# eggsbenedicto/DiffusionRenderer-ComfyUI

Measured on AMD Instinct MI355X. Metric: denoising_steps_per_sec, higher is better.
Workload: dtype bf16; 1 GPU; inverse pass, 57f x 576 x 1024 clip: EDM Euler step = 1 DiT forward (D=4096, 28 blocks, 32 heads) over S=18432 tokens, guidance 0; parallelism=sp1 (token bands; self-attention exchange: none), weights=random-init (hash generator), 7.2e9 params bf16

## Files before the change

diffusionrenderer-comfyui_amd/csrc/attention16.hip:

```cpp
#include "drn_common.h"
#include "drn_launchers.h"
#include "mx_quant.h"

#define QROWS 256
#define KVT 64
#define KBYTES (KVT * 256)
#define NKB 3
#define NVB 4
#ifndef RESCALE_THR
#define RESCALE_THR 6.0f
#endif

typedef const __attribute__((address_space(1))) void* gptr_t;
typedef __attribute__((address_space(3))) void* lptr_t;

template <bool MX>
__global__ __launch_bounds__(512, 2) void attention16_fwd_kernel(
    const bf16_t* __restrict__ Q, const bf16_t* __restrict__ Kp, const bf16_t* __restrict__ Vp, bf16_t* __restrict__ O,
    int heads, int64_t Sq, int64_t Sk_total, int64_t ldq, int64_t ldk, int64_t ldv, int64_t ldo, int64_t bsq, int64_t bsk,
    int64_t bsv, int64_t bso, float scale_log2e, int nqb, int total, int nsplit, int64_t kv_chunk,
    float* __restrict__ Opart, float* __restrict__ MLpart, uint8_t* __restrict__ OQ, uint8_t* __restrict__ OS, int64_t mx_bs) {
    __shared__ __attribute__((aligned(1024))) char smem[(NKB + NVB) * KBYTES];

    const int tid = threadIdx.x;
    const int lane = tid & 63;
    const int wave = __builtin_amdgcn_readfirstlane(tid >> 6);
    const int c = lane & 15, g = lane >> 4;

    int pid;
    {
        const int bid = blockIdx.x;
        const int q = total >> 3, r = total & 7, xcd = bid & 7;
        pid = (xcd < r ? xcd * (q + 1) : r * (q + 1) + (xcd - r) * q) + (bid >> 3);
    }
    const int qb = pid % nqb;
    const int rest = pid / nqb;
    const int split = rest % nsplit;
    const int bh = rest / nsplit;
    const int b = bh / heads, head = bh - b * heads;
    const int64_t q0 = (int64_t)qb * QROWS + wave * 32;
    const int64_t kv_begin = (int64_t)split * kv_chunk;
    const int64_t Sk = min(kv_chunk, Sk_total - kv_begin);

    const bf16_t* Qb = Q + b * bsq + (int64_t)head * 128;
    const bf16_t* Kb = Kp + b * bsk + kv_begin * ldk + (int64_t)head * 128;
    const bf16_t* Vb = Vp + b * bsv + kv_begin * ldv + (int64_t)head * 128;

    bf16x8_t qf[2][4];
#pragma unroll
    for (int qt = 0; qt < 2; ++qt) {
        int64_t qrow = q0 + 16 * qt + c;
        if (qrow > Sq - 1) qrow = Sq - 1;
        const bf16_t* qp = Qb + qrow * ldq + 8 * g;
#pragma unroll
        for (int ks = 0; ks < 4; ++ks) qf[qt][ks] = *reinterpret_cast<const bf16x8_t*>(qp + 32 * ks);
    }
#pragma unroll
    for (int qt = 0; qt < 2; ++qt)
#pragma unroll
        for (int ks = 0; ks < 4; ++ks) asm volatile("" : "+v"(qf[qt][ks]));

    int st_row[2], st_kc[2], st_vc[2];
#pragma unroll
    for (int i = 0; i < 2; ++i) {
        st_row[i] = 4 * (2 * wave + i) + (lane >> 4);
        const int cp = lane & 15;
        st_kc[i] = (cp ^ (st_row[i] & 15)) * 8;
        st_vc[i] = (cp ^ (((st_row[i] & 3) << 1) | (((st_row[i] >> 3) & 1) << 3))) * 8;
    }
    const int dma_off = wave * 2048;
    uint32_t kso[2], vso[2];
#pragma unroll
    for (int i = 0; i < 2; ++i) {
        kso[i] = 2u * (uint32_t)(st_row[i] * (int)ldk + st_kc[i]);
// ... 1 lines not shown
    }
    const int last_rows = (int)(Sk - (int64_t)((Sk - 1) / KVT) * KVT);
#define CLAMP_LAST_TILE()                                                                     \
    do {                                                                                      \
        _Pragma("unroll") for (int i = 0; i < 2; ++i) {                                       \
            const int r_ = min(st_row[i], last_rows - 1);                                     \
            kso[i] = 2u * (uint32_t)(r_ * (int)ldk + st_kc[i]);                               \
            vso[i] = 2u * (uint32_t)(r_ * (int)ldv + st_vc[i]);                               \
        }                                                                                     \
    } while (0)
#define DMA16(SRC, DST) __builtin_amdgcn_global_load_lds((gptr_t)(SRC), (lptr_t)(DST), 16, 0, 0)
#define DMA_PIECE_AT(P, KPTR, VPTR, KBUF, VBUF)                                               \
    do {                                                                                      \
        if ((P) & 1) DMA16((VPTR) + vso[(P) >> 1], smem + (NKB + (VBUF)) * KBYTES + dma_off + ((P) >> 1) * 1024); \
        else DMA16((KPTR) + kso[(P) >> 1], smem + (KBUF) * KBYTES + dma_off + ((P) >> 1) * 1024); \
    } while (0)
#define DMA_WAIT(N) asm volatile("s_waitcnt vmcnt(%0)" :: "i"(N) : "memory")
#define FENCE() __builtin_amdgcn_sched_barrier(0)
#define BARRIER()                                                                             \
    do {                                                                                      \
        FENCE();                                                                              \
        __builtin_amdgcn_s_barrier();                                                         \
        FENCE();                                                                              \
    } while (0)

    const uint32_t lds0 = (uint32_t)(uintptr_t)((lptr_t)smem);
    const int pc = (c & 3) | ((c & 4) << 1) | ((c & 8) >> 1);
    uint32_t ka[4];
#pragma unroll
    for (int ks = 0; ks < 4; ++ks) ka[ks] = lds0 + pc * 256 + (((4 * ks + g) ^ pc) << 4);
    const int vq = c >> 2, vp = c & 3;
    const int kap = ((g & 1) << 3) | ((g & 2) << 1);
    uint32_t va[8];
#pragma unroll
    for (int dt = 0; dt < 8; ++dt)
        va[dt] = lds0 + NKB * KBYTES + (kap + vq) * 256 + 32 * (dt ^ (vq | ((g & 1) << 2))) + 16 * (vp >> 1) + 8 * (vp & 1);

    f32x4_t acc[8][2];
#pragma unroll
    for (int dt = 0; dt < 8; ++dt)
#pragma unroll
        for (int qt = 0; qt < 2; ++qt) acc[dt][qt] = f32x4_t{0.f, 0.f, 0.f, 0.f};
    float m_run[2] = {-INFINITY, -INFINITY}, l_run[2] = {0.f, 0.f};
    f32x4_t lacc[2] = {f32x4_t{0.f, 0.f, 0.f, 0.f}, f32x4_t{0.f, 0.f, 0.f, 0.f}};
    bf16x8_t ones_frag;
#pragma unroll
    for (int i = 0; i < 8; ++i) ones_frag[i] = (short)0x3f80;
    asm volatile("" : "+v"(ones_frag));
    f32x4_t sacc[4][2];
    bf16x8_t pb[2][2] = {};

    bf16x8_t kring[8];
    struct vfrag_t { bf16x4_t lo, hi; } vring[8];
#define RD_K(F16, SLOT)                                                             \
    asm volatile("ds_read_b128 %0, %1 offset:%2" : "=v"(kring[SLOT]) : "v"(ka[(F16) & 3]), "i"(((F16) >> 2) * 4096) : "memory")
#define RD_V(F16, SLOT)                                              \
    asm volatile("ds_read_b64_tr_b16 %0, %2 offset:%3\n\tds_read_b64_tr_b16 %1, %2 offset:%4"                         \
                 : "=&v"(vring[SLOT].lo), "=&v"(vring[SLOT].hi)                                                       \
                 : "v"(va[(F16) & 7]), "i"((32 * ((F16) >> 3)) * 256), "i"((32 * ((F16) >> 3) + 16) * 256) : "memory")
#ifndef ATT16_TIE
#define ATT16_TIE 0
#endif
#if ATT16_TIE
#define WAIT_K(N, SLOT) asm volatile("s_waitcnt lgkmcnt(%1)" : "+v"(kring[SLOT]) : "i"(N) : "memory")
#define WAIT_V(N, SLOT) asm volatile("s_waitcnt lgkmcnt(%2)" : "+v"(vring[SLOT].lo), "+v"(vring[SLOT].hi) : "i"(N) : "memory")
#else
#define WAIT_K(N, SLOT) asm volatile("s_waitcnt lgkmcnt(%0)" :: "i"(N) : "memory")
#define WAIT_V(N, SLOT) asm volatile("s_waitcnt lgkmcnt(%0)" :: "i"(N) : "memory")
#endif
#define JOIN(X) __builtin_shufflevector(X.lo, X.hi, 0, 1, 2, 3, 4, 5, 6, 7)
#define MFMA16(A, B, C) __builtin_amdgcn_mfma_f32_16x16x32_bf16(A, B, C, 0, 0, 0)
#define ISSUE(F)                                                                              \
    do {                                                                                      \
        if ((F) < 16) RD_V(F, (F) & 7);                                                       \
        else if ((F) < 32) RD_K((F) - 16, (F) & 7);                                           \
        else RD_V((F) - 32, (F) & 7);                                                         \
    } while (0)
#define NV_(F) ((F) < 16 ? 2 : ((F) < 32 ? 1 : 2))
#define PEND(F) (NV_((F) + 1) + NV_((F) + 2) + NV_((F) + 3) + NV_((F) + 4) + NV_((F) + 5) + NV_((F) + 6) + NV_((F) + 7))
#ifndef ATT16_PAIR
#define ATT16_PAIR 0
#endif
#ifndef ATT16_DMA_IN_S
#define ATT16_DMA_IN_S 0
#endif
#ifndef ATT16_LSUM_MFMA
#define ATT16_LSUM_MFMA 1
#endif
#ifndef ATT16_PRIO
#define ATT16_PRIO 1
#endif
#ifndef ATT16_SPRIO
#define ATT16_SPRIO 0
#endif
#ifndef ATT16_BAR1
#define ATT16_BAR1 0
#endif
#ifndef ATT16_ABL
#define ATT16_ABL 0
#endif
#define PAIRED(F, PENDING) (ATT16_PAIR && !ATT16_TIE ? (((F) & 1) ? -1 : (PENDING) - NV_((F) + 1)) : (PENDING))
#define STEP_PV(F, PENDING, NEXT)                                                             \
    do {                                                                                      \
        if (PAIRED(F, PENDING) >= 0) WAIT_V(PAIRED(F, PENDING), (F) & 7);                     \
        FENCE();                                                                              \
        {                                                                                     \
            const bf16x8_t vf_ = JOIN(vring[(F) & 7]);                                        \
            acc[(F) & 7][0] = MFMA16(vf_, pb[(F) >> 3][0], acc[(F) & 7][0]);                  \
            acc[(F) & 7][1] = MFMA16(vf_, pb[(F) >> 3][1], acc[(F) & 7][1]);                  \
            if (ATT16_LSUM_MFMA && ((F) & 7) == 4) {        \
                lacc[0] = MFMA16(ones_frag, pb[(F) >> 3][0], lacc[0]);                        \
                lacc[1] = MFMA16(ones_frag, pb[(F) >> 3][1], lacc[1]);                        \
            }                                                                                 \
        }                                                                                     \
        if (NEXT) ISSUE((F) + 8);                                                             \
        FENCE();                                                                              \
    } while (0)
#define STEP_QK(F, PENDING)                                                                   \
    do {                                                                                      \
        if (PAIRED(F, PENDING) >= 0) WAIT_K(PAIRED(F, PENDING), (F) & 7);                     \
        FENCE();                                                                              \
        if ((((F) - 16) & 3) == 0) {                                                          \
            sacc[((F) - 16) >> 2][0] = MFMA16(kring[(F) & 7], qf[0][0], (f32x4_t{0.f, 0.f, 0.f, 0.f})); \
            sacc[((F) - 16) >> 2][1] = MFMA16(kring[(F) & 7], qf[1][0], (f32x4_t{0.f, 0.f, 0.f, 0.f})); \
        } else {                                                                              \
            sacc[((F) - 16) >> 2][0] = MFMA16(kring[(F) & 7], qf[0][((F) - 16) & 3], sacc[((F) - 16) >> 2][0]); \
            sacc[((F) - 16) >> 2][1] = MFMA16(kring[(F) & 7], qf[1][((F) - 16) & 3], sacc[((F) - 16) >> 2][1]); \
        }                                                                                     \
        ISSUE((F) + 8);                                                                       \
        FENCE();                                                                              \
    } while (0)
#define K_STEP(DELTA) do { _Pragma("unroll") for (int ks = 0; ks < 4; ++ks) ka[ks] += (DELTA); } while (0)
#define V_STEP(DELTA) do { _Pragma("unroll") for (int dt = 0; dt < 8; ++dt) va[dt] += (DELTA); } while (0)

#define QK_MASK(T)                                                                            \
    do {                                                                                      \
        if ((int64_t)((T) + 1) * KVT > Sk) {                                                  \
            const int64_t kbase = (int64_t)(T) * KVT + kap;                                   \
            _Pragma("unroll") for (int kt = 0; kt < 4; ++kt)                                  \
                _Pragma("unroll") for (int i = 0; i < 4; ++i)                                 \
                    if (kbase + 16 * kt + i >= Sk) { sacc[kt][0][i] = -INFINITY; sacc[kt][1][i] = -INFINITY; } \
        }                                                                                     \
    } while (0)

#define MAX3(A, B, C) __builtin_fmaxf(__builtin_fmaxf(A, B), C)
#define SOFTMAX_PHASE()                                                                       \
    do {                                                                                      \
        float mx[2];                                                                          \
        {    \
            float a0[2], a2[2];                                                               \
            _Pragma("unroll") for (int qt = 0; qt < 2; ++qt) {                                \
                float b0 = MAX3(sacc[0][qt][0], sacc[0][qt][1], sacc[0][qt][2]);              \
                float b1 = MAX3(sacc[0][qt][3], sacc[1][qt][0], sacc[1][qt][1]);              \
                float b2 = MAX3(sacc[1][qt][2], sacc[1][qt][3], sacc[2][qt][0]);              \
                float b3 = MAX3(sacc[2][qt][1], sacc[2][qt][2], sacc[2][qt][3]);              \
                float b4 = MAX3(sacc[3][qt][0], sacc[3][qt][1], sacc[3][qt][2]);              \
                a0[qt] = MAX3(b0, b1, sacc[3][qt][3]);                                        \
                a2[qt] = MAX3(b2, b3, b4);                                                    \
            }                                                                                 \
            uint32_t u0 = __float_as_uint(fmaxf(a0[0], a2[0])), u1 = __float_as_uint(fmaxf(a0[1], a2[1])); \
            auto s0 = __builtin_amdgcn_permlane32_swap(u0, u0, false, false);       \
            auto s1 = __builtin_amdgcn_permlane32_swap(u1, u1, false, false);                 \
            u0 = __float_as_uint(fmaxf(__uint_as_float(s0[0]), __uint_as_float(s0[1])));      \
            u1 = __float_as_uint(fmaxf(__uint_as_float(s1[0]), __uint_as_float(s1[1])));      \
            s0 = __builtin_amdgcn_permlane16_swap(u0, u0, false, false);            \
            s1 = __builtin_amdgcn_permlane16_swap(u1, u1, false, false);                      \
            mx[0] = fmaxf(__uint_as_float(s0[0]), __uint_as_float(s0[1]));                    \
            mx[1] = fmaxf(__uint_as_float(s1[0]), __uint_as_float(s1[1]));                    \
        }                                                                                     \
         \
        if (__any(mx[0] > m_thr[0] || mx[1] > m_thr[1])) {                                    \
            _Pragma("unroll") for (int qt = 0; qt < 2; ++qt) {                                \
                const float m_new = fmaxf(m_run[qt], mx[qt]);                                 \
                const float alpha = __builtin_amdgcn_exp2f((m_run[qt] - m_new) * scale_log2e); \
                m_run[qt] = m_new;                                                            \
                m_thr[qt] = m_new + thr_raw;                                                  \
                mcs[qt] = m_new * scale_log2e;                                                \
                l_run[qt] *= alpha;                                                           \
                lacc[qt] *= alpha;                                                            \
                _Pragma("unroll") for (int dt = 0; dt < 8; ++dt) acc[dt][qt] *= alpha;        \
            }                                                                                 \
        }                                                                                     \
        _Pragma("unroll") for (int qt = 0; qt < 2; ++qt) {                                    \
            const float mc = mcs[qt];                                                         \
            float ps[2] = {0.f, 0.f};                                                         \
            _Pragma("unroll") for (int s_ = 0; s_ < 2; ++s_) {                                \
                float p[8];                                                                   \
                _Pragma("unroll") for (int j = 0; j < 8; ++j) {                               \
                    if (ATT16_ABL & 1) p[j] = sacc[2 * s_ + (j >> 2)][qt][j & 3] * scale_log2e - mc;      \
                    else p[j] = __builtin_amdgcn_exp2f(sacc[2 * s_ + (j >> 2)][qt][j & 3] * scale_log2e - mc); \
                    if (!ATT16_LSUM_MFMA) ps[j & 1] += p[j];                                  \
                }                                                                             \
                union { bf16x8_t v; uint32_t u[4]; } cv;                                      \
                _Pragma("unroll") for (int i = 0; i < 4; ++i) cv.u[i] = pack_bf2(p[2 * i], p[2 * i + 1]); \
                pb[s_][qt] = cv.v;                                                            \
            }                                                                                 \
            if (!ATT16_LSUM_MFMA) l_run[qt] += ps[0] + ps[1];                                 \
        }                                                                                     \
    } while (0)

    const float thr_raw = RESCALE_THR / scale_log2e;
    float m_thr[2] = {-INFINITY, -INFINITY}, mcs[2] = {0.f, 0.f};
    const int nt = (int)((Sk + KVT - 1) / KVT);
    const int grp = wave >> 2;
    if (nt == 1 && last_rows < KVT) CLAMP_LAST_TILE();
    {
        const char* k0_ = reinterpret_cast<const char*>(Kb);
        const char* v0_ = reinterpret_cast<const char*>(Vb);
        DMA_PIECE_AT(0, k0_, v0_, 0, 0); DMA_PIECE_AT(1, k0_, v0_, 0, 0); DMA_PIECE_AT(2, k0_, v0_, 0, 0); DMA_PIECE_AT(3, k0_, v0_, 0, 0);
    }
    const int64_t ktile_bytes = (int64_t)KVT * ldk * 2, vtile_bytes = (int64_t)KVT * ldv * 2;
    if (nt > 1) {
        if (nt == 2 && last_rows < KVT) CLAMP_LAST_TILE();
        const char* k1_ = reinterpret_cast<const char*>(Kb) + ktile_bytes;
        const char* v1_ = reinterpret_cast<const char*>(Vb) + vtile_bytes;
        DMA_PIECE_AT(0, k1_, v1_, 1, 1); DMA_PIECE_AT(1, k1_, v1_, 1, 1); DMA_PIECE_AT(2, k1_, v1_, 1, 1); DMA_PIECE_AT(3, k1_, v1_, 1, 1);
    }
    DMA_WAIT(0);
    BARRIER();
    if (nt == 3 && last_rows < KVT) CLAMP_LAST_TILE();
    if (!ATT16_BAR1 && grp == 1) BARRIER();
    const char* kreq_p = reinterpret_cast<const char*>(Kb) + (int64_t)min(2, nt - 1) * ktile_bytes;
    const char* vreq_p = reinterpret_cast<const char*>(Vb) + (int64_t)min(2, nt - 1) * vtile_bytes;
    int kbuf = 0, vbuf = 0;
    int kreq = 2 % NKB, vreq = 2 % NVB;
#define REQ_PIECE_NOW(P)                                                                      \
    do {                                                                                      \
        if (!(ATT16_ABL & 4)) DMA_PIECE_AT(P, kreq_p, vreq_p, kreq, vreq);                    \
        FENCE();                                                                              \
    } while (0)
#define REQ_PIECE(P) do { if (!ATT16_DMA_IN_S) REQ_PIECE_NOW(P); } while (0)
#define AFTER_REQUESTS(T)                                                                     \
    do {                                                                                      \
        kreq = kreq == NKB - 1 ? 0 : kreq + 1;                                                \
        vreq = vreq == NVB - 1 ? 0 : vreq + 1;                                                \
        if ((T) + 3 == nt - 1 && last_rows < KVT) CLAMP_LAST_TILE();     \
        if (!(ATT16_ABL & 8) && (T) + 3 <= nt - 1) { kreq_p += ktile_bytes; vreq_p += vtile_bytes; }    \
    } while (0)
#define M_QK(T)                                                                               \
    do {                                                                                      \
        STEP_QK(16, PEND(16)); STEP_QK(17, PEND(17)); STEP_QK(18, PEND(18)); STEP_QK(19, PEND(19)); \
        REQ_PIECE(2);                                                                         \
        STEP_QK(20, PEND(20)); STEP_QK(21, PEND(21)); STEP_QK(22, PEND(22)); STEP_QK(23, PEND(23)); \
        K_STEP(kbuf == NKB - 1 ? -(NKB - 1) * KBYTES : KBYTES);                               \
        kbuf = kbuf == NKB - 1 ? 0 : kbuf + 1;                                                \
        STEP_QK(24, PEND(24)); STEP_QK(25, PEND(25)); STEP_QK(26, PEND(26)); STEP_QK(27, PEND(27)); \
        REQ_PIECE(3);                                                                         \
        STEP_QK(28, PEND(28)); STEP_QK(29, PEND(29)); STEP_QK(30, PEND(30)); STEP_QK(31, PEND(31)); \
        QK_MASK(T);                                                                           \
        if (!ATT16_DMA_IN_S) AFTER_REQUESTS(T);                                               \
        FENCE();                                                                              \
        __builtin_amdgcn_s_setprio(ATT16_SPRIO);                                              \
         \
        if (!ATT16_BAR1 || grp == 1) {                                                        \
            if (ATT16_DMA_IN_S) DMA_WAIT(0); else DMA_WAIT(4);                                \
            BARRIER();                                                                        \
        }                                                                                     \
    } while (0)
#define S_SEGMENT(T)                                                                          \
    do {                                                                                      \
        if (ATT16_DMA_IN_S) {                                                                 \
            REQ_PIECE_NOW(0); REQ_PIECE_NOW(1); REQ_PIECE_NOW(2); REQ_PIECE_NOW(3);           \
            AFTER_REQUESTS(T);                                                                \
        }                                                                                     \
        if (!(ATT16_ABL & 2)) SOFTMAX_PHASE();                                                \
        else { _Pragma("unroll") for (int kt = 0; kt < 4; ++kt) asm volatile("" :: "v"(sacc[kt][0]), "v"(sacc[kt][1])); } \
        FENCE();                                                                              \
         \
        asm volatile("" : "+v"(pb[0][0]), "+v"(pb[0][1]), "+v"(pb[1][0]), "+v"(pb[1][1]), "+v"(l_run[0]), "+v"(l_run[1]) :: "memory"); \
        if (!ATT16_BAR1) BARRIER();                                                           \
        else if (grp == 0) { DMA_WAIT(4); BARRIER(); }                                        \
    } while (0)

    __builtin_amdgcn_s_setprio(ATT16_PRIO);
    ISSUE(16); ISSUE(17); ISSUE(18); ISSUE(19); ISSUE(20); ISSUE(21); ISSUE(22); ISSUE(23);
    FENCE();
    REQ_PIECE(0);
    REQ_PIECE(1);
    M_QK(0);
    S_SEGMENT(0);
    for (int t = 1; t < nt; ++t) {
        __builtin_amdgcn_s_setprio(ATT16_PRIO);
        STEP_PV(0, PEND(0), 1); STEP_PV(1, PEND(1), 1); STEP_PV(2, PEND(2), 1); STEP_PV(3, PEND(3), 1);
        REQ_PIECE(0);
        STEP_PV(4, PEND(4), 1); STEP_PV(5, PEND(5), 1); STEP_PV(6, PEND(6), 1); STEP_PV(7, PEND(7), 1);
        V_STEP(vbuf == NVB - 1 ? -(NVB - 1) * KBYTES : KBYTES);
        vbuf = vbuf == NVB - 1 ? 0 : vbuf + 1;
        STEP_PV(8, PEND(8), 1); STEP_PV(9, PEND(9), 1); STEP_PV(10, PEND(10), 1); STEP_PV(11, PEND(11), 1);
        REQ_PIECE(1);
        STEP_PV(12, PEND(12), 1); STEP_PV(13, PEND(13), 1); STEP_PV(14, PEND(14), 1); STEP_PV(15, PEND(15), 1);
        M_QK(t);
        S_SEGMENT(t);
    }
    __builtin_amdgcn_s_setprio(ATT16_PRIO);
    STEP_PV(0, 14, 1); STEP_PV(1, 14, 1); STEP_PV(2, 14, 1); STEP_PV(3, 14, 1);
    STEP_PV(4, 14, 1); STEP_PV(5, 14, 1); STEP_PV(6, 14, 1); STEP_PV(7, 14, 1);
    STEP_PV(8, 14, 0); STEP_PV(9, 12, 0); STEP_PV(10, 10, 0); STEP_PV(11, 8, 0);
    STEP_PV(12, 6, 0); STEP_PV(13, 4, 0); STEP_PV(14, 2, 0); STEP_PV(15, 0, 0);
    __builtin_amdgcn_s_setprio(0);
    DMA_WAIT(0);
    if (!ATT16_BAR1 && grp == 0) BARRIER();

    float l_tot[2];
#pragma unroll
    for (int qt = 0; qt < 2; ++qt) {
        if (ATT16_LSUM_MFMA) {
            l_tot[qt] = lacc[qt][0];
        } else {
            float l = l_run[qt] + __shfl_xor(l_run[qt], 16, 64);
            l_tot[qt] = l + __shfl_xor(l, 32, 64);
        }
    }
    if (nsplit > 1) {
        const int nbatch = total / (nqb * heads * nsplit);
#pragma unroll
        for (int qt = 0; qt < 2; ++qt) {
            const int64_t qrow = q0 + 16 * qt + c;
            if (qrow < Sq) {
                const int64_t rowid = ((int64_t)split * nbatch + b) * Sq + qrow;
                float* op = Opart + rowid * ((int64_t)heads * 128) + (int64_t)head * 128 + 4 * g;
#pragma unroll
                for (int dt = 0; dt < 8; ++dt) *reinterpret_cast<f32x4_t*>(op + 16 * dt) = acc[dt][qt];
                if (g == 0) {
                    float2* ml = reinterpret_cast<float2*>(MLpart) + rowid * heads + head;
                    *ml = make_float2(m_run[qt], l_tot[qt]);
                }
            }
        }
        return;
    }
    __syncthreads();
    {
        char* ob = smem + wave * 8192;
#pragma unroll
        for (int qt = 0; qt < 2; ++qt) {
            const float inv = 1.0f / l_tot[qt];
            const int r = 16 * qt + c;
#pragma unroll
            for (int dt = 0; dt < 8; ++dt) {
                uint2 o;
                o.x = pack_bf2(acc[dt][qt][0] * inv, acc[dt][qt][1] * inv);
                o.y = pack_bf2(acc[dt][qt][2] * inv, acc[dt][qt][3] * inv);
                *reinterpret_cast<uint2*>(ob + r * 256 + (((2 * dt + (g >> 1)) ^ (r & 15)) << 4) + 8 * (g & 1)) = o;
            }
        }
        asm volatile("s_waitcnt lgkmcnt(0)" ::: "memory");
        const int oc = lane & 15;
        bf16_t* op = O + b * bso + (int64_t)head * 128 + oc * 8;
#pragma unroll
        for (int j = 0; j < 8; ++j) {
            const int row = 4 * j + (lane >> 4);
            const uint4 v = *reinterpret_cast<const uint4*>(ob + row * 256 + ((oc ^ (row & 15)) << 4));
            const int64_t qr = q0 + row;
            if (!MX) {
                if (qr < Sq) *reinterpret_cast<uint4*>(op + qr * ldo) = v;
            } else {
                uint32_t amax = max(max(mx_amax2(v.x), mx_amax2(v.y)), max(mx_amax2(v.z), mx_amax2(v.w)));
                amax = max(amax, (uint32_t)__shfl_xor((int)amax, 1, 64));
                amax = max(amax, (uint32_t)__shfl_xor((int)amax, 2, 64));
                const int e = mx_block_exp(amax);
                const float inv = mx_inv_scale(e);
                if (qr < Sq) {
                    const int64_t r = b * mx_bs + qr;
                    *reinterpret_cast<uint2*>(OQ + (r * heads + head) * 128 + oc * 8) = make_uint2(mx_pack4(v.x, v.y, inv), mx_pack4(v.z, v.w, inv));
                    if ((oc & 3) == 0) OS[(r * heads + head) * 4 + (oc >> 2)] = (uint8_t)(e + 127);
                    if (O) *reinterpret_cast<uint4*>(op + qr * ldo) = v;
                }
            }
        }
    }
}

void drn_attention16_launch(const void* q, const void* k, const void* v, void* o, int heads, int64_t Sq, int64_t Sk, int64_t ldq,
                            int64_t ldk, int64_t ldv, int64_t ldo, int64_t bsq, int64_t bsk, int64_t bsv, int64_t bso,
                            float scale_log2e, int nqb, int64_t total, int nsplit, int64_t kv_chunk, float* opart, float* mlpart,
                            hipStream_t st, void* oq, void* os, int64_t mx_bs) {
    if (oq)
        attention16_fwd_kernel<true><<<dim3((unsigned)total, 1, 1), dim3(512), 0, st>>>(
            (const bf16_t*)q, (const bf16_t*)k, (const bf16_t*)v, (bf16_t*)o, heads, Sq, Sk, ldq, ldk, ldv, ldo, bsq, bsk, bsv, bso,
            scale_log2e, nqb, (int)total, nsplit, kv_chunk, opart, mlpart, (uint8_t*)oq, (uint8_t*)os, mx_bs);
    else
        attention16_fwd_kernel<false><<<dim3((unsigned)total, 1, 1), dim3(512), 0, st>>>(
            (const bf16_t*)q, (const bf16_t*)k, (const bf16_t*)v, (bf16_t*)o, heads, Sq, Sk, ldq, ldk, ldv, ldo, bsq, bsk, bsv, bso,
            scale_log2e, nqb, (int)total, nsplit, kv_chunk, opart, mlpart, nullptr, nullptr, 0);
}
```

diffusionrenderer-comfyui_amd/native.py:

```python
import ctypes
import os
from ctypes import POINTER, Structure, c_char_p, c_double, c_float, c_int, c_int32, c_int64, c_void_p

import torch

_LIB = None
_LIB_NAME = "libdrn.so"

EPI_NONE, EPI_GELU, EPI_GATE_RES = 0, 1, 2
ACT_NONE, ACT_SILU = 0, 1

_P, _I, _L, _F = c_void_p, c_int, c_int64, c_float

SUB_FA, SUB_CA, SUB_MLP = 0, 1, 2


class DitSub(Structure):
    _fields_ = [("kind", c_int32), ("site", c_int32), ("ca_index", c_int32), ("reserved", c_int32),
                ("w_a", c_void_p), ("w_b", c_void_p), ("qn", c_void_p), ("kn", c_void_p),
                ("s_a", c_void_p), ("s_b", c_void_p)]


class DitForwardArgs(Structure):
    _fields_ = [("struct_bytes", c_int64), ("S", c_int64), ("B", c_int64), ("D", c_int64), ("hidden", c_int64),
# ... 25 lines not shown
    "drn_timer_destroy": [_P],
    "drn_timer_count": [_P],
    "drn_timer_seen": [_P, _I],
    "drn_timer_read": [_P, _I, POINTER(c_int), POINTER(c_float), POINTER(c_double), POINTER(c_double)],
    "drn_abi_version": [],
    "drn_error_string": [_I],
    "drn_gemm_bf16": [_P, _P, _P, _L, _L, _L, _L, _L, _L, _I, _P, _P, _L, _L, _P],
    "drn_gemm_bf16_blocked": [_P, _P, _P, _L, _L, _L, _L, _L, _L, _I, _P, _P, _L, _L, _L, _L, _L, _L, _P],
    "drn_gemm_bf16_splitk": [_P, _P, _P, _L, _L, _L, _L, _L, _L, _I, _P, _P, _L, _L, _I, _P, _P],
    "drn_gemm_splitk_workspace_bytes": [_L, _L, _I],
    "drn_gemm_bf16_f32out": [_P, _P, _P, _L, _L, _L, _L, _L, _P],
    "drn_gemm_bf16_splitk_partials": [_P, _P, _L, _L, _L, _L, _L, _L, _I, _P, _P],
    "drn_splitk_gate_res_ln_modulate": [_P, _I, _P, _P, _P, _P, _P, _P, _L, _L, _L, _F, _P],
    "drn_gemm_splitk_choice": [_L, _L, _L],
    "drn_gemm_tile_choice": [_L, _L],
    "drn_gemm_force_tile": [_I],
    "drn_gemm_force_res_prefetch": [_I],
    "drn_gemm_tall_force_shape": [_I],
    "drn_mx_quant_bf16": [_P, _L, _L, _L, _P, _P, _P],
    "drn_mx_quant_calls": [_I],
    "drn_gemm_mxfp8_gelu_mx": [_P, _P, _P, _P, _P, _P, _L, _L, _L, _L, _P],
    "drn_ln_modulate_mx": [_P, _P, _P, _P, _P, _P, _P, _L, _L, _L, _F, _P],
    "drn_splitk_gate_res_ln_modulate_mx": [_P, _I, _P, _P, _P, _P, _P, _P, _P, _P, _L, _L, _L, _F, _P],
    "drn_attention_bf16_mx": [_P, _P, _P, _P, _P, _P, _I, _I, _L, _L, _L, _L, _L, _L, _L, _L, _L, _L, _F, _P],
    "drn_attention_splitkv_bf16_mx": [_P, _P, _P, _P, _P, _P, _I, _I, _L, _L, _L, _L, _L, _L, _L, _L, _L, _L, _F, _I, _P, _P],
    "drn_attention_mx_available": [],
    "drn_attention_mxfp8_params": [POINTER(c_int), POINTER(c_float), POINTER(c_int)],
    "drn_attention_mxfp8_choice": [_I, _L],
    "drn_attention_mxfp8_force": [_I],
    "drn_qk_norm_rope_mx": [_P, _P, _P, _P, _P, _P, _P, _P, _P, _P, _L, _I, _L, _L, _L, _L, _F, _I, _P],
    "drn_mx_quant_vt": [_P, _P, _P, _I, _I, _L, _L, _L, _P],
    "drn_attention_mxfp8": [_P, _P, _P, _P, _P, _P, _P, _P, _P, _I, _I, _L, _L, _L, _L, _L, _L, _F, _P],
    "drn_attention_splitkv_mxfp8": [_P, _P, _P, _P, _P, _P, _P, _P, _P, _I, _I, _L, _L, _L, _L, _L, _L, _F, _I, _P, _P],
    "drn_dit_forward_mx_attn_bytes": [_L, _L, _L],
    "drn_dit_forward_mx_attn_layout": [_L, _L, _L, POINTER(c_int64)],
    "drn_gemm_mxfp8": [_P, _P, _P, _P, _P, _L, _L, _L, _L, _I, _P, _P, _L, _L, _P],
    "drn_gemm_mxfp8_blocked": [_P, _P, _P, _P, _P, _L, _L, _L, _L, _I, _P, _P, _L, _L, _L, _L, _L, _L, _P],
    "drn_gemm_mxfp8_splitk_choice": [_L, _L, _L],
    "drn_gemm_mxfp8_splitk": [_P, _P, _P, _P, _P, _L, _L, _L, _L, _I, _P, _P, _L, _L, _I, _P, _P],
    "drn_gemm_mxfp8_splitk_partials": [_P, _P, _P, _P, _L, _L, _L, _L, _I, _P, _P],
    "drn_gemm_mxfp8_force_small_m": [_I],
    "drn_gemm_mxfp8_tall_force_shape": [_I],
    "drn_gemv_bf16": [_P, _P, _P, _L, _L, _I, _I, _L, _L, _L, _L, _L, _P, _L, _L, _P, _L, _L, _I, _P],
    "drn_ln_modulate": [_P, _P, _P, _P, _P, _L, _L, _L, _F, _P],
    "drn_ln_force_kernel": [_I],
    "drn_bcast_add": [_P, _P, _L, _L, _L, _P],
    "drn_permute_021": [_P, _P, _L, _L, _L, _P],
    "drn_rmsnorm": [_P, _P, _P, _L, _L, _F, _P],
    "drn_qk_norm_rope": [_P, _P, _P, _P, _P, _P, _L, _I, _L, _L, _L, _L, _F, _P],
    "drn_attention_bf16": [_P, _P, _P, _P, _I, _I, _L, _L, _L, _L, _L, _L, _L, _L, _L, _L, _F, _P],
    "drn_attention_splitkv_bf16": [_P, _P, _P, _P, _I, _I, _L, _L, _L, _L, _L, _L, _L, _L, _L, _L, _F, _I, _P, _P],
    "drn_attention_splitkv_workspace_bytes": [_I, _I, _L, _I],
    "drn_attention_force_shape16": [_I],
    "drn_patchify_concat": [_P, _P, _P, _I, _I, _I, _I, _I, _I, _I, _I, _I, _L, _P],
    "drn_unpatchify": [_P, _L, _P, _I, _I, _I, _I, _I, _I, _I, _P],
    "drn_edm_scale_input": [_P, _P, _L, _F, _P],
    "drn_edm_step": [_P, _P, _P, _L, _F, _F, _F, _F, _P],
    "drn_cfg_combine": [_P, _P, _P, _L, _F, _P],
    "drn_postprocess_u8": [_P, _P, _I, _I, _I, _I, _I, _P],
}
_RESTYPES = {"drn_error_string": c_char_p, "drn_attention_splitkv_workspace_bytes": c_int64,
             "drn_gemm_splitk_workspace_bytes": c_int64, "drn_dit_forward_gemm_workspace_bytes": c_int64,
             "drn_dit_forward_attn_workspace_bytes": c_int64, "drn_dit_forward_mx_act_bytes": c_int64,
             "drn_dit_forward_mx_u_bytes": c_int64, "drn_mx_quant_calls": c_int64, "drn_dit_forward_mx_attn_bytes": c_int64,
             "drn_dit_forward_mx_gemm_workspace_bytes": c_int64, "drn_dit_forward_args_bytes": c_int64, "drn_dit_sub_bytes": c_int64, "drn_timer_create": c_void_p, "drn_timer_destroy": None,
             "drn_ln_force_kernel": None, "drn_attention_force_shape16": None}


def library_path() -> str:
    return os.path.join(os.path.dirname(os.path.abspath(__file__)), _LIB_NAME)


def load_library():
    global _LIB
    if _LIB is not None:
        return _LIB
    path = library_path()
    if not os.path.exists(path):
        raise RuntimeError(f"{path} not found: build it with `python __graft_entry__.py` (hipcc --offload-arch=gfx950); "
                           "there is no CPU / eager fallback for the hot path")
    lib = ctypes.CDLL(path)
    for name, argtypes in SIGNATURES.items():
        fn = getattr(lib, name)
        fn.argtypes = argtypes
        fn.restype = _RESTYPES.get(name, c_int)
    if lib.drn_abi_version() != 1:
        raise RuntimeError("libdrn.so ABI version mismatch")
    if lib.drn_dit_forward_args_bytes() != ctypes.sizeof(DitForwardArgs) or lib.drn_dit_sub_bytes() != ctypes.sizeof(DitSub):
        raise RuntimeError("libdrn.so: drn_dit_forward_args / drn_dit_sub layout differs from the ctypes mirror in native.py")
    _LIB = lib
    return lib


def _check(code: int, what: str):
    if code != 0:
        msg = load_library().drn_error_string(code)
        raise RuntimeError(f"{what} failed ({code}): {msg.decode() if msg else '?'}")


def _ptr(t):
    if t is None:
        return None
    assert t.is_cuda, "device tensor required"
    return t.data_ptr()


def _stream():
    return torch.cuda.current_stream().cuda_stream


def _bf16(*ts):
    for t in ts:
        if t is not None:
            assert t.dtype == torch.bfloat16, f"bf16 tensor required, got {t.dtype}"


class KernelTimer:

    def __init__(self, names=("gemm", "attention"), sample_every=1):
# ... 568 lines not shown
```

include/drn.h:

```cpp
#ifndef DRN_H
#define DRN_H

#include <stdint.h>

#ifdef __cplusplus
extern "C" {
#endif

#define DRN_OK 0
#define DRN_EINVAL (-1)

#define DRN_ABI_VERSION 1

#define DRN_EPI_NONE 0
#define DRN_EPI_GELU 1
#define DRN_EPI_GATE_RES 2

#define DRN_ACT_NONE 0
#define DRN_ACT_SILU 1

int drn_abi_version(void);
const char* drn_error_string(int code);

int drn_gemm_bf16(const void* A, const void* W, void* C, int64_t M, int64_t N, int64_t K,
// ... 30 lines not shown
int drn_gemm_mxfp8(const void* A, const void* SA, const void* W, const void* SW, void* C, int64_t M, int64_t N, int64_t K,
                   int64_t ldc, int epilogue, const void* gate, const void* residual, int64_t ldr, int64_t rows_per_batch,
                   void* stream);
int drn_gemm_mxfp8_blocked(const void* A, const void* SA, const void* W, const void* SW, void* C, int64_t M, int64_t N, int64_t K,
                           int64_t ldc, int epilogue, const void* gate, const void* residual, int64_t ldr, int64_t rows_per_batch,
                           int64_t a_block_cols, int64_t a_block_stride, int64_t c_block_cols, int64_t c_block_stride,
                           void* stream);
int drn_gemm_mxfp8_splitk_choice(int64_t M, int64_t N, int64_t K);
int drn_gemm_mxfp8_splitk(const void* A, const void* SA, const void* W, const void* SW, void* C, int64_t M, int64_t N, int64_t K,
                          int64_t ldc, int epilogue, const void* gate, const void* residual, int64_t ldr, int64_t rows_per_batch,
                          int splits, void* workspace, void* stream);
int drn_gemm_mxfp8_splitk_partials(const void* A, const void* SA, const void* W, const void* SW, int64_t M, int64_t N, int64_t K,
                                   int64_t rows_per_batch, int splits, void* workspace, void* stream);
int drn_gemm_mxfp8_force_small_m(int on);
int drn_gemm_mxfp8_tall_force_shape(int shape);

int drn_gemv_bf16(const void* x, const void* W, void* y, int64_t N, int64_t K,
                  int groups, int batch,
                  int64_t x_gstride, int64_t x_bstride, int64_t w_gstride,
                  int64_t y_gstride, int64_t y_bstride,
                  const void* add, int64_t add_gstride, int64_t add_bstride,
                  const void* mul, int64_t mul_gstride, int64_t mul_bstride,
                  int act, void* stream);

int drn_ln_modulate(void* x, const void* add_vec, const void* shift, const void* scale, void* h,
                    int64_t rows, int64_t D, int64_t rows_per_batch, float eps, void* stream);
int drn_ln_modulate_mx(void* x, const void* add_vec, const void* shift, const void* scale, void* h, void* hq, void* hs,
                       int64_t rows, int64_t D, int64_t rows_per_batch, float eps, void* stream);
int drn_splitk_gate_res_ln_modulate(const void* partials, int splits, void* x, const void* gate, const void* add_vec,
                                    const void* shift, const void* scale, void* h, int64_t rows, int64_t D,
                                    int64_t rows_per_batch, float eps, void* stream);
int drn_splitk_gate_res_ln_modulate_mx(const void* partials, int splits, void* x, const void* gate, const void* add_vec,
                                       const void* shift, const void* scale, void* h, void* hq, void* hs, int64_t rows, int64_t D,
                                       int64_t rows_per_batch, float eps, void* stream);
void drn_ln_force_kernel(int which);

int drn_bcast_add(void* x, const void* vec, int64_t rows, int64_t D, int64_t rows_per_batch, void* stream);

int drn_permute_021(const void* x, void* y, int64_t A, int64_t B, int64_t C, void* stream);

int drn_rmsnorm(const void* x, const void* w, void* y, int64_t rows, int64_t D, float eps, void* stream);

int drn_qk_norm_rope(void* q, void* k, const void* wq, const void* wk, const void* cos, const void* sin,
                     int64_t tokens, int heads, int64_t ldq, int64_t ldk, int64_t tokens_per_batch,
                     int64_t pos_offset, float eps, void* stream);

int drn_attention_bf16(const void* q, const void* k, const void* v, void* o,
                       int batch, int heads, int64_t Sq, int64_t Sk,
                       int64_t ldq, int64_t ldk, int64_t ldv, int64_t ldo,
                       int64_t bsq, int64_t bsk, int64_t bsv, int64_t bso,
                       float scale, void* stream);

void drn_attention_force_shape16(int on);

int drn_attention_splitkv_bf16(const void* q, const void* k, const void* v, void* o,
                               int batch, int heads, int64_t Sq, int64_t Sk,
                               int64_t ldq, int64_t ldk, int64_t ldv, int64_t ldo,
                               int64_t bsq, int64_t bsk, int64_t bsv, int64_t bso,
                               float scale, int nsplit, void* workspace, void* stream);
int64_t drn_attention_splitkv_workspace_bytes(int batch, int heads, int64_t Sq, int nsplit);

int drn_attention_bf16_mx(const void* q, const void* k, const void* v, void* o, void* oq, void* os,
                          int batch, int heads, int64_t Sq, int64_t Sk,
                          int64_t ldq, int64_t ldk, int64_t ldv, int64_t ldo,
                          int64_t bsq, int64_t bsk, int64_t bsv, int64_t bso,
                          float scale, void* stream);
int drn_attention_splitkv_bf16_mx(const void* q, const void* k, const void* v, void* o, void* oq, void* os,
                                  int batch, int heads, int64_t Sq, int64_t Sk,
                                  int64_t ldq, int64_t ldk, int64_t ldv, int64_t ldo,
                                  int64_t bsq, int64_t bsk, int64_t bsv, int64_t bso,
                                  float scale, int nsplit, void* workspace, void* stream);
int drn_attention_mx_available(void);

int drn_attention_mxfp8_params(int* key_tile, float* rescale_thr, int* pexp);
int drn_attention_mxfp8_choice(int heads, int64_t S);
int drn_attention_mxfp8_force(int on);
int drn_qk_norm_rope_mx(void* q, void* k, const void* wq, const void* wk, const void* cos, const void* sin,
                        void* qq, void* qs, void* kq, void* ks,
                        int64_t tokens, int heads, int64_t ldq, int64_t ldk, int64_t tokens_per_batch,
                        int64_t pos_offset, float eps, int write_bf16, void* stream);
int drn_mx_quant_vt(const void* v, void* vt, void* vs, int batch, int heads, int64_t Sk, int64_t ldv, int64_t bsv, void* stream);
int drn_attention_mxfp8(const void* qq, const void* qs, const void* kq, const void* ks, const void* vt, const void* vs,
                        void* o, void* oq, void* os, int batch, int heads, int64_t Sq, int64_t Sk,
                        int64_t q_bs, int64_t k_bs, int64_t ldo, int64_t bso, float scale, void* stream);
int drn_attention_splitkv_mxfp8(const void* qq, const void* qs, const void* kq, const void* ks, const void* vt, const void* vs,
                                void* o, void* oq, void* os, int batch, int heads, int64_t Sq, int64_t Sk,
                                int64_t q_bs, int64_t k_bs, int64_t ldo, int64_t bso, float scale,
                                int nsplit, void* workspace, void* stream);

int drn_attention_plan(int heads, int64_t Sq, int64_t Sk, int64_t* plan);

#define DRN_SUB_FA 0
#define DRN_SUB_CA 1
#define DRN_SUB_MLP 2
typedef struct drn_dit_sub {
    int32_t kind;
    int32_t site;
    int32_t ca_index;
    int32_t reserved;
    const void* w_a;
    const void* w_b;
    const void* qn;
    const void* kn;
    const void* s_a;
    const void* s_b;
} drn_dit_sub;
// ... 92 lines not shown
```

Measured before the change: 3.494 steps/s.

## Unroll attention16 KV loop by four with static ring-buffer LDS offsets

Raises the K ring from 3 to 4 buffers so both K and V rings have period 4, then unrolls the main KV-tile loop by four. Each unrolled tile uses compile-time LDS offsets folded into ds_read immediates and fixed DMA slot indices instead of runtime pointer and index rotation. This is meant to remove per-tile scalar and vector address arithmetic and ring-index bookkeeping. The tail mask computation is also simplified to 32-bit. The extra K buffer enlarges LDS use, which may affect the two-blocks-per-CU occupancy, and a runtime switch keeps the old dynamic path.

```diff
diff --git a/diffusionrenderer-comfyui_amd/csrc/attention16.hip b/diffusionrenderer-comfyui_amd/csrc/attention16.hip
--- a/diffusionrenderer-comfyui_amd/csrc/attention16.hip
+++ b/diffusionrenderer-comfyui_amd/csrc/attention16.hip
@@ -5,7 +5,12 @@
 #define QROWS 256
 #define KVT 64
 #define KBYTES (KVT * 256)
-#define NKB 3
+#ifndef ATT16_STATIC_RING
+#define ATT16_STATIC_RING 1
+#endif
+#ifndef NKB
+#define NKB (ATT16_STATIC_RING ? 4 : 3)
+#endif
 #define NVB 4
 #ifndef RESCALE_THR
 #define RESCALE_THR 6.0f
@@ -19,7 +24,8 @@
     const bf16_t* __restrict__ Q, const bf16_t* __restrict__ Kp, const bf16_t* __restrict__ Vp, bf16_t* __restrict__ O,
     int heads, int64_t Sq, int64_t Sk_total, int64_t ldq, int64_t ldk, int64_t ldv, int64_t ldo, int64_t bsq, int64_t bsk,
     int64_t bsv, int64_t bso, float scale_log2e, int nqb, int total, int nsplit, int64_t kv_chunk,
-    float* __restrict__ Opart, float* __restrict__ MLpart, uint8_t* __restrict__ OQ, uint8_t* __restrict__ OS, int64_t mx_bs) {
+    float* __restrict__ Opart, float* __restrict__ MLpart, uint8_t* __restrict__ OQ, uint8_t* __restrict__ OS, int64_t mx_bs,
+    int force_dynamic) {
     __shared__ __attribute__((aligned(1024))) char smem[(NKB + NVB) * KBYTES];
 
     const int tid = threadIdx.x;
@@ -127,12 +133,12 @@
 
     bf16x8_t kring[8];
     struct vfrag_t { bf16x4_t lo, hi; } vring[8];
-#define RD_K(F16, SLOT)                                                             \
-    asm volatile("ds_read_b128 %0, %1 offset:%2" : "=v"(kring[SLOT]) : "v"(ka[(F16) & 3]), "i"(((F16) >> 2) * 4096) : "memory")
-#define RD_V(F16, SLOT)                                              \
+#define RD_K(F16, SLOT, OFF)                                                        \
+    asm volatile("ds_read_b128 %0, %1 offset:%2" : "=v"(kring[SLOT]) : "v"(ka[(F16) & 3]), "i"((OFF) + ((F16) >> 2) * 4096) : "memory")
+#define RD_V(F16, SLOT, OFF)                                         \
     asm volatile("ds_read_b64_tr_b16 %0, %2 offset:%3\n\tds_read_b64_tr_b16 %1, %2 offset:%4"                         \
                  : "=&v"(vring[SLOT].lo), "=&v"(vring[SLOT].hi)                                                       \
-                 : "v"(va[(F16) & 7]), "i"((32 * ((F16) >> 3)) * 256), "i"((32 * ((F16) >> 3) + 16) * 256) : "memory")
+                 : "v"(va[(F16) & 7]), "i"((OFF) + (32 * ((F16) >> 3)) * 256), "i"((OFF) + (32 * ((F16) >> 3) + 16) * 256) : "memory")
 #ifndef ATT16_TIE
 #define ATT16_TIE 0
 #endif
@@ -145,11 +151,11 @@
 #endif
 #define JOIN(X) __builtin_shufflevector(X.lo, X.hi, 0, 1, 2, 3, 4, 5, 6, 7)
 #define MFMA16(A, B, C) __builtin_amdgcn_mfma_f32_16x16x32_bf16(A, B, C, 0, 0, 0)
-#define ISSUE(F)                                                                              \
-    do {                                                                                      \
-        if ((F) < 16) RD_V(F, (F) & 7);                                                       \
-        else if ((F) < 32) RD_K((F) - 16, (F) & 7);                                           \
-        else RD_V((F) - 32, (F) & 7);                                                         \
+#define ISSUE(F, OFF)                                                                         \
+    do {                                                                                      \
+        if ((F) < 16) RD_V(F, (F) & 7, OFF);                                                  \
+        else if ((F) < 32) RD_K((F) - 16, (F) & 7, OFF);                                      \
+        else RD_V((F) - 32, (F) & 7, OFF);                                                    \
     } while (0)
 #define NV_(F) ((F) < 16 ? 2 : ((F) < 32 ? 1 : 2))
 #define PEND(F) (NV_((F) + 1) + NV_((F) + 2) + NV_((F) + 3) + NV_((F) + 4) + NV_((F) + 5) + NV_((F) + 6) + NV_((F) + 7))
@@ -175,7 +181,7 @@
 #define ATT16_ABL 0
 #endif
 #define PAIRED(F, PENDING) (ATT16_PAIR && !ATT16_TIE ? (((F) & 1) ? -1 : (PENDING) - NV_((F) + 1)) : (PENDING))
-#define STEP_PV(F, PENDING, NEXT)                                                             \
+#define STEP_PV(F, PENDING, NEXT, OFF)                                                        \
     do {                                                                                      \
         if (PAIRED(F, PENDING) >= 0) WAIT_V(PAIRED(F, PENDING), (F) & 7);                     \
         FENCE();                                                                              \
@@ -188,10 +194,10 @@
                 lacc[1] = MFMA16(ones_frag, pb[(F) >> 3][1], lacc[1]);                        \
             }                                                                                 \
         }                                                                                     \
-        if (NEXT) ISSUE((F) + 8);                                                             \
-        FENCE();                                                                              \
-    } while (0)
-#define STEP_QK(F, PENDING)                                                                   \
+        if (NEXT) ISSUE((F) + 8, OFF);                                                        \
+        FENCE();                                                                              \
+    } while (0)
+#define STEP_QK(F, PENDING, OFF)                                                              \
     do {                                                                                      \
         if (PAIRED(F, PENDING) >= 0) WAIT_K(PAIRED(F, PENDING), (F) & 7);                     \
         FENCE();                                                                              \
@@ -202,7 +208,7 @@
             sacc[((F) - 16) >> 2][0] = MFMA16(kring[(F) & 7], qf[0][((F) - 16) & 3], sacc[((F) - 16) >> 2][0]); \
             sacc[((F) - 16) >> 2][1] = MFMA16(kring[(F) & 7], qf[1][((F) - 16) & 3], sacc[((F) - 16) >> 2][1]); \
         }                                                                                     \
-        ISSUE((F) + 8);                                                                       \
+        ISSUE((F) + 8, OFF);                                                                  \
         FENCE();                                                                              \
     } while (0)
 #define K_STEP(DELTA) do { _Pragma("unroll") for (int ks = 0; ks < 4; ++ks) ka[ks] += (DELTA); } while (0)
@@ -211,10 +217,10 @@
 #define QK_MASK(T)                                                                            \
     do {                                                                                      \
         if ((int64_t)((T) + 1) * KVT > Sk) {                                                  \
-            const int64_t kbase = (int64_t)(T) * KVT + kap;                                   \
+            const int rem_ = (int)(Sk - (int64_t)(T) * KVT);      \
             _Pragma("unroll") for (int kt = 0; kt < 4; ++kt)                                  \
                 _Pragma("unroll") for (int i = 0; i < 4; ++i)                                 \
-                    if (kbase + 16 * kt + i >= Sk) { sacc[kt][0][i] = -INFINITY; sacc[kt][1][i] = -INFINITY; } \
+                    if (kap >= rem_ - (16 * kt + i)) { sacc[kt][0][i] = -INFINITY; sacc[kt][1][i] = -INFINITY; } \
         }                                                                                     \
     } while (0)
 
@@ -299,31 +305,35 @@
     const char* vreq_p = reinterpret_cast<const char*>(Vb) + (int64_t)min(2, nt - 1) * vtile_bytes;
     int kbuf = 0, vbuf = 0;
     int kreq = 2 % NKB, vreq = 2 % NVB;
-#define REQ_PIECE_NOW(P)                                                                      \
-    do {                                                                                      \
-        if (!(ATT16_ABL & 4)) DMA_PIECE_AT(P, kreq_p, vreq_p, kreq, vreq);                    \
-        FENCE();                                                                              \
-    } while (0)
-#define REQ_PIECE(P) do { if (!ATT16_DMA_IN_S) REQ_PIECE_NOW(P); } while (0)
-#define AFTER_REQUESTS(T)                                                                     \
-    do {                                                                                      \
-        kreq = kreq == NKB - 1 ? 0 : kreq + 1;                                                \
-        vreq = vreq == NVB - 1 ? 0 : vreq + 1;                                                \
+#define REQ_PIECE_NOW(P, KREQ, VREQ)                                                          \
+    do {                                                                                      \
+        if (!(ATT16_ABL & 4)) DMA_PIECE_AT(P, kreq_p, vreq_p, KREQ, VREQ);                    \
+        FENCE();                                                                              \
+    } while (0)
+#define REQ_PIECE(P, KREQ, VREQ) do { if (!ATT16_DMA_IN_S) REQ_PIECE_NOW(P, KREQ, VREQ); } while (0)
+#define AFTER_REQUESTS(T, DYN)                                                                \
+    do {                                                                                      \
+        if (DYN) {                                                                            \
+            kreq = kreq == NKB - 1 ? 0 : kreq + 1;                                            \
+            vreq = vreq == NVB - 1 ? 0 : vreq + 1;                                            \
+        }                                                                                     \
         if ((T) + 3 == nt - 1 && last_rows < KVT) CLAMP_LAST_TILE();     \
         if (!(ATT16_ABL & 8) && (T) + 3 <= nt - 1) { kreq_p += ktile_bytes; vreq_p += vtile_bytes; }    \
     } while (0)
-#define M_QK(T)                                                                               \
-    do {                                                                                      \
-        STEP_QK(16, PEND(16)); STEP_QK(17, PEND(17)); STEP_QK(18, PEND(18)); STEP_QK(19, PEND(19)); \
-        REQ_PIECE(2);                                                                         \
-        STEP_QK(20, PEND(20)); STEP_QK(21, PEND(21)); STEP_QK(22, PEND(22)); STEP_QK(23, PEND(23)); \
-        K_STEP(kbuf == NKB - 1 ? -(NKB - 1) * KBYTES : KBYTES);                               \
-        kbuf = kbuf == NKB - 1 ? 0 : kbuf + 1;                                                \
-        STEP_QK(24, PEND(24)); STEP_QK(25, PEND(25)); STEP_QK(26, PEND(26)); STEP_QK(27, PEND(27)); \
-        REQ_PIECE(3);                                                                         \
-        STEP_QK(28, PEND(28)); STEP_QK(29, PEND(29)); STEP_QK(30, PEND(30)); STEP_QK(31, PEND(31)); \
+#define M_QK(T, KO, VO, KREQ, VREQ, DYN)                                                      \
+    do {                                                                                      \
+        STEP_QK(16, PEND(16), KO); STEP_QK(17, PEND(17), KO); STEP_QK(18, PEND(18), KO); STEP_QK(19, PEND(19), KO); \
+        REQ_PIECE(2, KREQ, VREQ);                                                             \
+        STEP_QK(20, PEND(20), KO); STEP_QK(21, PEND(21), KO); STEP_QK(22, PEND(22), KO); STEP_QK(23, PEND(23), KO); \
+        if (DYN) {                                                                            \
+            K_STEP(kbuf == NKB - 1 ? -(NKB - 1) * KBYTES : KBYTES);                           \
+            kbuf = kbuf == NKB - 1 ? 0 : kbuf + 1;                                            \
+        }                                                                                     \
+        STEP_QK(24, PEND(24), VO); STEP_QK(25, PEND(25), VO); STEP_QK(26, PEND(26), VO); STEP_QK(27, PEND(27), VO); \
+        REQ_PIECE(3, KREQ, VREQ);                                                             \
+        STEP_QK(28, PEND(28), VO); STEP_QK(29, PEND(29), VO); STEP_QK(30, PEND(30), VO); STEP_QK(31, PEND(31), VO); \
         QK_MASK(T);                                                                           \
-        if (!ATT16_DMA_IN_S) AFTER_REQUESTS(T);                                               \
+        if (!ATT16_DMA_IN_S) AFTER_REQUESTS(T, DYN);                                          \
         FENCE();                                                                              \
         __builtin_amdgcn_s_setprio(ATT16_SPRIO);                                              \
          \
@@ -332,11 +342,11 @@
             BARRIER();                                                                        \
         }                                                                                     \
     } while (0)
-#define S_SEGMENT(T)                                                                          \
+#define S_SEGMENT(T, KREQ, VREQ, DYN)                                                         \
     do {                                                                                      \
         if (ATT16_DMA_IN_S) {                                                                 \
-            REQ_PIECE_NOW(0); REQ_PIECE_NOW(1); REQ_PIECE_NOW(2); REQ_PIECE_NOW(3);           \
-            AFTER_REQUESTS(T);                                                                \
+            REQ_PIECE_NOW(0, KREQ, VREQ); REQ_PIECE_NOW(1, KREQ, VREQ); REQ_PIECE_NOW(2, KREQ, VREQ); REQ_PIECE_NOW(3, KREQ, VREQ); \
+            AFTER_REQUESTS(T, DYN);                                                           \
         }                                                                                     \
         if (!(ATT16_ABL & 2)) SOFTMAX_PHASE();                                                \
         else { _Pragma("unroll") for (int kt = 0; kt < 4; ++kt) asm volatile("" :: "v"(sacc[kt][0]), "v"(sacc[kt][1])); } \
@@ -346,32 +356,51 @@
         if (!ATT16_BAR1) BARRIER();                                                           \
         else if (grp == 0) { DMA_WAIT(4); BARRIER(); }                                        \
     } while (0)
+#define TILE(T, VPO, KO, VO, KREQ, VREQ, DYN)                                                 \
+    do {                                                                                      \
+        __builtin_amdgcn_s_setprio(ATT16_PRIO);                                               \
+        STEP_PV(0, PEND(0), 1, VPO); STEP_PV(1, PEND(1), 1, VPO); STEP_PV(2, PEND(2), 1, VPO); STEP_PV(3, PEND(3), 1, VPO); \
+        REQ_PIECE(0, KREQ, VREQ);                                                             \
+        STEP_PV(4, PEND(4), 1, VPO); STEP_PV(5, PEND(5), 1, VPO); STEP_PV(6, PEND(6), 1, VPO); STEP_PV(7, PEND(7), 1, VPO); \
+        if (DYN) {                                                                            \
+            V_STEP(vbuf == NVB - 1 ? -(NVB - 1) * KBYTES : KBYTES);                           \
+            vbuf = vbuf == NVB - 1 ? 0 : vbuf + 1;                                            \
+        }                                                                                     \
+        STEP_PV(8, PEND(8), 1, KO); STEP_PV(9, PEND(9), 1, KO); STEP_PV(10, PEND(10), 1, KO); STEP_PV(11, PEND(11), 1, KO); \
+        REQ_PIECE(1, KREQ, VREQ);                                                             \
+        STEP_PV(12, PEND(12), 1, KO); STEP_PV(13, PEND(13), 1, KO); STEP_PV(14, PEND(14), 1, KO); STEP_PV(15, PEND(15), 1, KO); \
+        M_QK(T, KO, VO, KREQ, VREQ, DYN);                                                     \
+        S_SEGMENT(T, KREQ, VREQ, DYN);                                                        \
+    } while (0)
+#define TILE_STATIC(T, R) TILE(T, (((R) + 3) & 3) * KBYTES, (R) * KBYTES, (R) * KBYTES, ((R) + 2) & 3, ((R) + 2) & 3, 0)
 
     __builtin_amdgcn_s_setprio(ATT16_PRIO);
-    ISSUE(16); ISSUE(17); ISSUE(18); ISSUE(19); ISSUE(20); ISSUE(21); ISSUE(22); ISSUE(23);
+    ISSUE(16, 0); ISSUE(17, 0); ISSUE(18, 0); ISSUE(19, 0); ISSUE(20, 0); ISSUE(21, 0); ISSUE(22, 0); ISSUE(23, 0);
     FENCE();
-    REQ_PIECE(0);
-    REQ_PIECE(1);
-    M_QK(0);
-    S_SEGMENT(0);
-    for (int t = 1; t < nt; ++t) {
-        __builtin_amdgcn_s_setprio(ATT16_PRIO);
-        STEP_PV(0, PEND(0), 1); STEP_PV(1, PEND(1), 1); STEP_PV(2, PEND(2), 1); STEP_PV(3, PEND(3), 1);
-        REQ_PIECE(0);
-        STEP_PV(4, PEND(4), 1); STEP_PV(5, PEND(5), 1); STEP_PV(6, PEND(6), 1); STEP_PV(7, PEND(7), 1);
-        V_STEP(vbuf == NVB - 1 ? -(NVB - 1) * KBYTES : KBYTES);
-        vbuf = vbuf == NVB - 1 ? 0 : vbuf + 1;
-        STEP_PV(8, PEND(8), 1); STEP_PV(9, PEND(9), 1); STEP_PV(10, PEND(10), 1); STEP_PV(11, PEND(11), 1);
-        REQ_PIECE(1);
-        STEP_PV(12, PEND(12), 1); STEP_PV(13, PEND(13), 1); STEP_PV(14, PEND(14), 1); STEP_PV(15, PEND(15), 1);
-        M_QK(t);
-        S_SEGMENT(t);
-    }
+    REQ_PIECE(0, kreq, vreq);
+    REQ_PIECE(1, kreq, vreq);
+    M_QK(0, 0, 0, kreq, vreq, 1);
+    S_SEGMENT(0, kreq, vreq, 1);
+    int t = 1;
+#if ATT16_STATIC_RING
+    static_assert(NKB == 4 && NVB == 4, "the static trips want both rings at period 4");
+    if (!force_dynamic && nt >= 5) {
+        K_STEP(-KBYTES);
+        for (; t + 4 <= nt; t += 4) {
+            TILE_STATIC(t, 1);
+            TILE_STATIC(t + 1, 2);
+            TILE_STATIC(t + 2, 3);
+            TILE_STATIC(t + 3, 0);
+        }
+        K_STEP(KBYTES);
+    }
+#endif
+    for (; t < nt; ++t) TILE(t, 0, 0, 0, kreq, vreq, 1);
     __builtin_amdgcn_s_setprio(ATT16_PRIO);
-    STEP_PV(0, 14, 1); STEP_PV(1, 14, 1); STEP_PV(2, 14, 1); STEP_PV(3, 14, 1);
-    STEP_PV(4, 14, 1); STEP_PV(5, 14, 1); STEP_PV(6, 14, 1); STEP_PV(7, 14, 1);
-    STEP_PV(8, 14, 0); STEP_PV(9, 12, 0); STEP_PV(10, 10, 0); STEP_PV(11, 8, 0);
-    STEP_PV(12, 6, 0); STEP_PV(13, 4, 0); STEP_PV(14, 2, 0); STEP_PV(15, 0, 0);
+    STEP_PV(0, 14, 1, 0); STEP_PV(1, 14, 1, 0); STEP_PV(2, 14, 1, 0); STEP_PV(3, 14, 1, 0);
+    STEP_PV(4, 14, 1, 0); STEP_PV(5, 14, 1, 0); STEP_PV(6, 14, 1, 0); STEP_PV(7, 14, 1, 0);
+    STEP_PV(8, 14, 0, 0); STEP_PV(9, 12, 0, 0); STEP_PV(10, 10, 0, 0); STEP_PV(11, 8, 0, 0);
+    STEP_PV(12, 6, 0, 0); STEP_PV(13, 4, 0, 0); STEP_PV(14, 2, 0, 0); STEP_PV(15, 0, 0, 0);
     __builtin_amdgcn_s_setprio(0);
     DMA_WAIT(0);
     if (!ATT16_BAR1 && grp == 0) BARRIER();
@@ -446,16 +475,20 @@
     }
 }
 
+static int g_att16_dynamic = 0;
+extern "C" void drn_attention16_force_dynamic(int on) { g_att16_dynamic = on; }
+
 void drn_attention16_launch(const void* q, const void* k, const void* v, void* o, int heads, int64_t Sq, int64_t Sk, int64_t ldq,
                             int64_t ldk, int64_t ldv, int64_t ldo, int64_t bsq, int64_t bsk, int64_t bsv, int64_t bso,
                             float scale_log2e, int nqb, int64_t total, int nsplit, int64_t kv_chunk, float* opart, float* mlpart,
                             hipStream_t st, void* oq, void* os, int64_t mx_bs) {
+    const int dyn = g_att16_dynamic != 0;
     if (oq)
         attention16_fwd_kernel<true><<<dim3((unsigned)total, 1, 1), dim3(512), 0, st>>>(
             (const bf16_t*)q, (const bf16_t*)k, (const bf16_t*)v, (bf16_t*)o, heads, Sq, Sk, ldq, ldk, ldv, ldo, bsq, bsk, bsv, bso,
-            scale_log2e, nqb, (int)total, nsplit, kv_chunk, opart, mlpart, (uint8_t*)oq, (uint8_t*)os, mx_bs);
+            scale_log2e, nqb, (int)total, nsplit, kv_chunk, opart, mlpart, (uint8_t*)oq, (uint8_t*)os, mx_bs, dyn);
     else
         attention16_fwd_kernel<false><<<dim3((unsigned)total, 1, 1), dim3(512), 0, st>>>(
             (const bf16_t*)q, (const bf16_t*)k, (const bf16_t*)v, (bf16_t*)o, heads, Sq, Sk, ldq, ldk, ldv, ldo, bsq, bsk, bsv, bso,
-            scale_log2e, nqb, (int)total, nsplit, kv_chunk, opart, mlpart, nullptr, nullptr, 0);
+            scale_log2e, nqb, (int)total, nsplit, kv_chunk, opart, mlpart, nullptr, nullptr, 0, dyn);
 }
diff --git a/diffusionrenderer-comfyui_amd/native.py b/diffusionrenderer-comfyui_amd/native.py
--- a/diffusionrenderer-comfyui_amd/native.py
+++ b/diffusionrenderer-comfyui_amd/native.py
@@ -101,6 +101,7 @@
     "drn_attention_splitkv_bf16": [_P, _P, _P, _P, _I, _I, _L, _L, _L, _L, _L, _L, _L, _L, _L, _L, _F, _I, _P, _P],
     "drn_attention_splitkv_workspace_bytes": [_I, _I, _L, _I],
     "drn_attention_force_shape16": [_I],
+    "drn_attention16_force_dynamic": [_I],
     "drn_patchify_concat": [_P, _P, _P, _I, _I, _I, _I, _I, _I, _I, _I, _I, _L, _P],
     "drn_unpatchify": [_P, _L, _P, _I, _I, _I, _I, _I, _I, _I, _P],
     "drn_edm_scale_input": [_P, _P, _L, _F, _P],
@@ -113,7 +114,8 @@
              "drn_dit_forward_attn_workspace_bytes": c_int64, "drn_dit_forward_mx_act_bytes": c_int64,
              "drn_dit_forward_mx_u_bytes": c_int64, "drn_mx_quant_calls": c_int64, "drn_dit_forward_mx_attn_bytes": c_int64,
              "drn_dit_forward_mx_gemm_workspace_bytes": c_int64, "drn_dit_forward_args_bytes": c_int64, "drn_dit_sub_bytes": c_int64, "drn_timer_create": c_void_p, "drn_timer_destroy": None,
-             "drn_ln_force_kernel": None, "drn_attention_force_shape16": None}
+             "drn_ln_force_kernel": None, "drn_attention_force_shape16": None,
+             "drn_attention16_force_dynamic": None}
 
 
 def library_path() -> str:
diff --git a/include/drn.h b/include/drn.h
--- a/include/drn.h
+++ b/include/drn.h
@@ -106,6 +106,8 @@
                        float scale, void* stream);
 
 void drn_attention_force_shape16(int on);
+
+void drn_attention16_force_dynamic(int on);
 
 int drn_attention_splitkv_bf16(const void* q, const void* k, const void* v, void* o,
                                int batch, int heads, int64_t Sq, int64_t Sk,
```

Result: no change. 3.515 steps/s (median of 6 runs) (+0.6%).
